# ICLDisco/parsec

Measured on NVIDIA H100. Metric: tasks/s, higher is better.
Workload: dtype i32

## Files before the change

include/pb2_engine.h:

```cpp
#ifndef PB2_ENGINE_H
#define PB2_ENGINE_H

#include <stddef.h>
#include <stdint.h>

#ifdef __cplusplus
extern "C" {
#endif

#define PB2_SUCCESS                   0
#define PB2_ERROR                    -1
#define PB2_ERR_OUT_OF_RESOURCE      -2
#define PB2_ERR_NOT_FOUND            -3
#define PB2_ERR_BAD_PARAM            -4
#define PB2_ERR_EXISTS               -5
#define PB2_ERR_NOT_IMPLEMENTED      -6
#define PB2_ERR_NOT_SUPPORTED        -7
#define PB2_ERR_VALUE_OUT_OF_BOUNDS  -8
#define PB2_ERR_TRUNCATE             -9
#define PB2_ERR_DEVICE              -10

#define PB2_FLOW_ACCESS_NONE   0x00
#define PB2_FLOW_ACCESS_READ   0x04
#define PB2_FLOW_ACCESS_WRITE  0x08
// ... 56 lines not shown
} pb2_tile_t;

#define PB2_SRC_HOST 0
#define PB2_SRC_PEER 1
#define PB2_SRC_PUSH 2

#define PB2_TILE_INVALID   0
#define PB2_TILE_STAGING   1
#define PB2_TILE_VALID     2

typedef struct pb2_engine_params_s {
    int32_t  workers_per_sm;
    int32_t  threads;
    int32_t  max_workers;
    int32_t  stage_mode;
    int32_t  queue_policy;
    int32_t  timeout_ms;
    int32_t  gemm_mode;
    int32_t  part_bytes;
    int32_t  read_groups;
    int32_t  fuse_readers;
} pb2_engine_params_t;

typedef struct pb2_engine_info_s {
    int32_t  cuda_device;
    int32_t  sm_count;
    int32_t  cc_major, cc_minor;
    int32_t  nworkers;
    int32_t  nworkers_gemm;
    int32_t  can_map_host;
    int32_t  reserved;
    uint64_t total_mem;
    uint64_t free_mem;
} pb2_engine_info_t;

typedef struct pb2_window_stats_s {
    uint64_t tasks_retired;
    uint64_t bytes_h2d;
    uint64_t bytes_d2d;
    uint64_t bytes_d2h;
    uint64_t stage_ins;
    uint64_t body_errors;
    float    kernel_ms;
    float    reset_ms;
} pb2_window_stats_t;

typedef struct pb2_engine_s pb2_engine_t;
typedef struct pb2_window_s pb2_window_t;

int  pb2_engine_create(pb2_engine_t** engine, int cuda_device, const pb2_engine_params_t* params);
int  pb2_engine_destroy(pb2_engine_t* engine);
int  pb2_engine_info(pb2_engine_t* engine, pb2_engine_info_t* info);
const char* pb2_engine_last_error(pb2_engine_t* engine);

int  pb2_engine_malloc(pb2_engine_t* engine, size_t bytes, void** dev_ptr);
int  pb2_engine_free(pb2_engine_t* engine, void* dev_ptr);
int  pb2_engine_host_register(pb2_engine_t* engine, void* host_ptr, size_t bytes, void** dev_alias);
int  pb2_engine_host_unregister(pb2_engine_t* engine, void* host_ptr);
int  pb2_engine_memcpy_h2d(pb2_engine_t* engine, void* dev, const void* host, size_t bytes);
int  pb2_engine_prefetch_h2d(pb2_engine_t* engine, void* dev, size_t dev_pitch, const void* host, size_t host_pitch,
                             size_t width_bytes, size_t rows);
int  pb2_engine_memcpy_d2h(pb2_engine_t* engine, void* host, const void* dev, size_t bytes);
int  pb2_engine_synchronize(pb2_engine_t* engine);
int  pb2_engine_set_stream(pb2_engine_t* engine, void* cuda_stream);
void* pb2_engine_get_stream(pb2_engine_t* engine);

int  pb2_engine_copy_batch(pb2_engine_t* engine, void* const* dst, const void* const* src, const uint64_t* bytes, int32_t n);

int  pb2_engine_ipc_export(pb2_engine_t* engine, void* dev_ptr, unsigned char handle[64]);
int  pb2_engine_ipc_open(pb2_engine_t* engine, const unsigned char handle[64], void** dev_ptr);
int  pb2_engine_ipc_close(pb2_engine_t* engine, void* dev_ptr);
int  pb2_engine_enable_peer(pb2_engine_t* engine, int peer_cuda_device);
int  pb2_body_launch(void* cuda_stream, int body, int nb_args, void* const* ptrs, const uint64_t* bytes,
                     const int32_t* iparam3, float fparam);
int  pb2_body_launch_errors(uint64_t* errors, int reset);
int  pb2_engine_set_shared_windows(pb2_engine_t* engine, int on, const int32_t* next_rs_begin);
int  pb2_engine_set_part_bytes(pb2_engine_t* engine, int32_t part_bytes);
int  pb2_engine_set_window_trace(pb2_engine_t* engine, int on);
int  pb2_engine_set_stage_slice_bytes(pb2_engine_t* engine, int32_t bytes);

#define PB2_IMAGE_PTX   1
#define PB2_IMAGE_CUBIN 2
int  pb2_engine_link_bodies(pb2_engine_t* engine, const void* image, size_t bytes, int format, uint32_t sliceable);
int  pb2_engine_link_bodies_checked(pb2_engine_t* engine, const void* image, size_t bytes, int format, uint32_t sliceable,
                                    uint32_t checked);
#define PB2_LINK_GEMM_WINDOWS 0x1u
#define PB2_LINK_READERS(mask) ((uint32_t)(mask) << 8)
#define PB2_LINK_READER_GROUPS(mask) ((uint32_t)(mask) << 16)
// ... 89 lines not shown
```

parsec_b200/_lib.py:

```python
import ctypes as C
import os

import numpy as np

_HERE = os.path.dirname(os.path.abspath(__file__))
LIB_PATH = os.environ.get("PB2_LIB_PATH") or os.path.join(_HERE, "libparsec_b200.so")

PB2_SUCCESS = 0
PB2_ERROR = -1
PB2_ERR_OUT_OF_RESOURCE = -2
PB2_ERR_NOT_FOUND = -3
PB2_ERR_BAD_PARAM = -4
PB2_ERR_EXISTS = -5
PB2_ERR_NOT_IMPLEMENTED = -6
PB2_ERR_NOT_SUPPORTED = -7
PB2_ERR_VALUE_OUT_OF_BOUNDS = -8
PB2_ERR_TRUNCATE = -9
PB2_ERR_DEVICE = -10

ERR_NAMES = {
    0: "PB2_SUCCESS", -1: "PB2_ERROR", -2: "PB2_ERR_OUT_OF_RESOURCE", -3: "PB2_ERR_NOT_FOUND",
    -4: "PB2_ERR_BAD_PARAM", -5: "PB2_ERR_EXISTS", -6: "PB2_ERR_NOT_IMPLEMENTED",
    -7: "PB2_ERR_NOT_SUPPORTED", -8: "PB2_ERR_VALUE_OUT_OF_BOUNDS", -9: "PB2_ERR_TRUNCATE",
    -10: "PB2_ERR_DEVICE",
}

ACCESS_NONE, ACCESS_READ, ACCESS_WRITE, ACCESS_RW, FLOW_PUSHOUT = 0x00, 0x04, 0x08, 0x0C, 0x40

BODY_NOP, BODY_FILL_I32, BODY_CHECK_I32, BODY_INCR_I32, BODY_ADD_IOTA_I32 = 0, 1, 2, 3, 4
BODY_SCALE_I32, BODY_IOTA_I32, BODY_COPY, BODY_FILL_F32, BODY_CHECK_F32 = 5, 6, 7, 8, 9
BODY_INCR_F32, BODY_AXPY_F32, BODY_MEMSET_U8, BODY_ADD_AT_I32, BODY_GEMM_BF16 = 10, 11, 12, 13, 16
BODY_LINKED_0, BODY_LINKED_7 = 20, 27
IMAGE_PTX, IMAGE_CUBIN = 1, 2
LINK_GEMM_WINDOWS = 0x1


def LINK_READERS(mask):
    return mask << 8


def LINK_READER_GROUPS(mask):
    return mask << 16


def LINK_GEMM_BODIES(mask):
    return mask << 24

TASK_DEPS_MASK = 0x01
TILE_INVALID, TILE_STAGING, TILE_VALID = 0, 1, 2
SRC_HOST, SRC_PEER = 0, 1
MAX_FLOWS = 4

TASK_DTYPE = np.dtype([
    ("dep_goal", "<i4"), ("succ_begin", "<i4"), ("succ_count", "<i4"), ("priority", "<i4"),
    ("body", "u1"), ("nb_flows", "u1"), ("flags", "u1"), ("class_id", "u1"),
    ("tile", "<i4", (4,)), ("access", "u1", (4,)),
    ("iparam", "<i4", (3,)), ("fparam", "<f4"), ("locals", "<i4", (2,)),
], align=False)
assert TASK_DTYPE.itemsize == 64

TILE_DTYPE = np.dtype([
    ("dev_ptr", "<u8"), ("src_ptr", "<u8"), ("bytes", "<u4"), ("state", "<i4"),
    ("version", "<u4"), ("src_kind", "<i4"),
], align=False)
assert TILE_DTYPE.itemsize == 32

PART_WAITED_INPUT, PART_RETIRED = 1, 2
PART_TRACE_DTYPE = np.dtype([
    ("t_pop_ns", "<u8"), ("t_in_ns", "<u8"), ("t_exec_ns", "<u8"), ("t_out_ns", "<u8"),
    ("in_bytes", "<u8"), ("out_bytes", "<u8"), ("task", "<i4"), ("part", "<u2"), ("nparts", "<u2"),
    ("smid", "<u4"), ("flags", "<u4"),
], align=False)
assert PART_TRACE_DTYPE.itemsize == 64

BODY_ARGS_DTYPE = np.dtype([
    ("flow", "<u8", (4,)), ("bytes", "<u4", (4,)), ("elem0", "<u4"), ("part", "<u4"),
    ("iparam", "<i4", (3,)), ("fparam", "<f4"),
], align=True)
assert BODY_ARGS_DTYPE.itemsize == 72


def succ_make(task, flow=0):
    return (np.uint32(flow) << np.uint32(27)) | np.uint32(task)


class EngineParams(C.Structure):
    _fields_ = [("workers_per_sm", C.c_int32), ("threads", C.c_int32), ("max_workers", C.c_int32),
                ("stage_mode", C.c_int32), ("queue_policy", C.c_int32), ("timeout_ms", C.c_int32),
                ("gemm_mode", C.c_int32), ("part_bytes", C.c_int32), ("read_groups", C.c_int32),
                ("fuse_readers", C.c_int32)]


class EngineInfo(C.Structure):
    _fields_ = [("cuda_device", C.c_int32), ("sm_count", C.c_int32), ("cc_major", C.c_int32),
                ("cc_minor", C.c_int32), ("nworkers", C.c_int32), ("nworkers_gemm", C.c_int32),
                ("can_map_host", C.c_int32), ("reserved", C.c_int32),
                ("total_mem", C.c_uint64), ("free_mem", C.c_uint64)]


class WindowStats(C.Structure):
    _fields_ = [("tasks_retired", C.c_uint64), ("bytes_h2d", C.c_uint64), ("bytes_d2d", C.c_uint64),
                ("bytes_d2h", C.c_uint64), ("stage_ins", C.c_uint64), ("body_errors", C.c_uint64),
                ("kernel_ms", C.c_float), ("reset_ms", C.c_float)]


class WindowHandle(C.Structure):
    _fields_ = [("dep", C.c_ubyte * 64), ("ring", C.c_ubyte * 64), ("ctl", C.c_ubyte * 64), ("tiles", C.c_ubyte * 64),
                ("cap_mask", C.c_uint32), ("ntasks", C.c_int32), ("entry_kind", C.c_int32), ("ntiles", C.c_int32)]


PUSH_DTYPE = np.dtype([("dst", np.uint64), ("bytes", np.uint32), ("src_tile", np.int32), ("rank", np.int32), ("desc", np.int32),
                       ("pad", np.int32, (2,))])
assert PUSH_DTYPE.itemsize == 32


class PartitionSizes(C.Structure):
    _fields_ = [("ntasks", C.c_int32), ("nsucc", C.c_int32), ("ntiles", C.c_int32), ("nready", C.c_int32),
                ("nremote", C.c_int32), ("nslots", C.c_int32), ("slab_bytes", C.c_uint64)]


class Pb2Error(RuntimeError):
    def __init__(self, rc, what, detail=""):
        self.rc = rc
        super().__init__(f"{what}: {ERR_NAMES.get(rc, rc)} {detail}".strip())


_lib = None

ENGINE_SYMBOLS = [
    "pb2_engine_create", "pb2_engine_destroy", "pb2_engine_info", "pb2_engine_last_error",
    "pb2_engine_malloc", "pb2_engine_free", "pb2_engine_host_register", "pb2_engine_host_unregister",
    "pb2_engine_memcpy_h2d", "pb2_engine_prefetch_h2d", "pb2_engine_memcpy_d2h", "pb2_engine_synchronize", "pb2_engine_set_stream", "pb2_engine_get_stream", "pb2_engine_copy_batch", "pb2_engine_ipc_export", "pb2_engine_ipc_open",
    "pb2_engine_ipc_close", "pb2_engine_enable_peer", "pb2_body_launch", "pb2_body_launch_errors", "pb2_engine_set_shared_windows", "pb2_engine_set_part_bytes", "pb2_engine_set_window_trace", "pb2_engine_set_stage_slice_bytes", "pb2_window_export", "pb2_window_set_remote", "pb2_window_task_entries",
    "pb2_window_arm", "pb2_window_start",
    "pb2_window_create", "pb2_window_destroy", "pb2_window_launch", "pb2_window_wait",
    "pb2_window_results", "pb2_window_trace", "pb2_window_part_trace",
    "pb2_partition_create", "pb2_partition_sizes", "pb2_partition_get", "pb2_partition_destroy", "pb2_partition_error",
    "pb2_partition_set_push", "pb2_partition_push_count", "pb2_partition_get_push", "pb2_window_set_push",
    "pb2_engine_link_bodies", "pb2_engine_link_bodies_checked", "pb2_engine_linked_info",
    "pb2_engine_link_bodies_ex", "pb2_engine_linked_gemm_info",
]


def load():
    global _lib
    if _lib is not None:
        return _lib
    if not os.path.exists(LIB_PATH):
        raise ImportError(
            f"{LIB_PATH} is missing: run `make` (or __graft_entry__.build()) first. "
            "parsec_b200 has no CPU fallback.")
    lib = C.CDLL(LIB_PATH)
    vp, i32, u64 = C.c_void_p, C.c_int32, C.c_uint64
    P = C.POINTER
    lib.pb2_engine_create.argtypes = [P(vp), C.c_int, P(EngineParams)]
    lib.pb2_engine_destroy.argtypes = [vp]
    lib.pb2_engine_info.argtypes = [vp, P(EngineInfo)]
    lib.pb2_engine_last_error.argtypes = [vp]
    lib.pb2_engine_last_error.restype = C.c_char_p
    lib.pb2_engine_malloc.argtypes = [vp, C.c_size_t, P(vp)]
    lib.pb2_engine_free.argtypes = [vp, vp]
    lib.pb2_engine_host_register.argtypes = [vp, vp, C.c_size_t, P(vp)]
    lib.pb2_engine_host_unregister.argtypes = [vp, vp]
    lib.pb2_engine_memcpy_h2d.argtypes = [vp, vp, vp, C.c_size_t]
    lib.pb2_engine_memcpy_d2h.argtypes = [vp, vp, vp, C.c_size_t]
    lib.pb2_engine_synchronize.argtypes = [vp]
    lib.pb2_engine_set_stream.argtypes = [vp, vp]
    lib.pb2_engine_copy_batch.argtypes = [vp, vp, vp, vp, i32]
    lib.pb2_engine_ipc_export.argtypes = [vp, vp, vp]
    lib.pb2_engine_ipc_open.argtypes = [vp, vp, P(vp)]
    lib.pb2_engine_ipc_close.argtypes = [vp, vp]
    lib.pb2_engine_enable_peer.argtypes = [vp, C.c_int]
    lib.pb2_body_launch.argtypes = [vp, C.c_int, C.c_int, vp, vp, vp, C.c_float]
    lib.pb2_body_launch_errors.argtypes = [vp, C.c_int]
    lib.pb2_engine_set_shared_windows.argtypes = [vp, C.c_int, vp]
    lib.pb2_window_task_entries.argtypes = [vp, vp]
    lib.pb2_engine_set_part_bytes.argtypes = [vp, i32]
    lib.pb2_engine_set_window_trace.argtypes = [vp, C.c_int]
    lib.pb2_window_trace.argtypes = [vp, vp, vp, vp, vp]
    lib.pb2_window_part_trace.argtypes = [vp, vp, i32, P(i32)]
    lib.pb2_engine_set_stage_slice_bytes.argtypes = [vp, i32]
    lib.pb2_engine_link_bodies.argtypes = [vp, C.c_char_p, C.c_size_t, C.c_int, C.c_uint32]
    lib.pb2_engine_link_bodies_checked.argtypes = [vp, C.c_char_p, C.c_size_t, C.c_int, C.c_uint32, C.c_uint32]
    lib.pb2_engine_linked_info.argtypes = [vp, P(i32), P(i32), P(i32), P(i32)]
    lib.pb2_engine_link_bodies_ex.argtypes = [vp, C.c_char_p, C.c_size_t, C.c_int, C.c_uint32, C.c_uint32, C.c_uint32]
    lib.pb2_engine_linked_gemm_info.argtypes = [vp, P(i32), P(i32), P(i32), P(i32)]
    lib.pb2_window_export.argtypes = [vp, vp]
    lib.pb2_window_set_remote.argtypes = [vp, i32, i32, vp, vp, vp, vp, i32]
    lib.pb2_partition_set_push.argtypes = [vp, C.c_int]
    lib.pb2_partition_push_count.argtypes = [vp, i32, vp]
    lib.pb2_partition_get_push.argtypes = [vp, i32, vp, vp, vp]
    lib.pb2_window_set_push.argtypes = [vp, vp, vp, i32]
    lib.pb2_window_arm.argtypes = [vp]
# ... 20 lines not shown
```

parsec_b200/csrc/pb2_engine.cu:

```cuda
#include <cuda_runtime.h>
#include <cuda.h>
#include <stdio.h>
#include <stdlib.h>
#include <string.h>
#include <string>
#include <vector>
#include <mutex>
#include <map>
#include <algorithm>
#include <type_traits>

#include "../../include/pb2_engine.h"
#include "pb2_sched.cuh"
#include "pb2_hbm.cuh"
#include "pb2_gemm.cuh"

namespace pb2 {

__global__ void pb2_window_reset_kernel(Win2Dev g, const pb2_tile_t* tiles_init,
                                        const int32_t* ready, int32_t nready) {
    const size_t gid = (size_t)blockIdx.x * blockDim.x + threadIdx.x;
    const size_t gsz = (size_t)gridDim.x * blockDim.x;
    for (size_t i = gid; i < (size_t)g.nunits; i += gsz) { g.udep[i] = g.units[i].dep_goal; g.parts_left[i] = g.units[i].nparts; }
    if (g.trace.parts)
// ... 206 lines not shown
static int read_part_records(pb2_window_t* w, std::vector<pb2_part_trace_t>& out) {
    pb2_engine_t* e = w->e;
    std::vector<pb2_part_trace_t> rec((size_t)w->shape.part_records);
    out.clear();
    if (rec.empty()) return PB2_SUCCESS;
    PB2_CUDA(e, cudaSetDevice(e->cuda_device));
    PB2_CUDA(e, cudaMemcpy(rec.data(), run_desc(w, w->cur).trace.parts, rec.size() * sizeof(pb2_part_trace_t), cudaMemcpyDeviceToHost));
    out.reserve(rec.size());
    for (const PartEntity& pe : w->part_entities)
        for (int32_t p = 0; p < pe.nparts; ++p) {
            out.push_back(rec[(size_t)(pe.base + p)]);
            out.back().task = pe.lead; out.back().part = (uint16_t)p; out.back().nparts = (uint16_t)pe.nparts;
        }
    return PB2_SUCCESS;
}

extern "C" const unsigned char pb2_linked_engine_image[], pb2_linked_engine_image_end[];
extern "C" const unsigned char pb2_linked_gemm_image[], pb2_linked_gemm_image_end[];
extern "C" const unsigned char pb2_linked_engine_groups_image[], pb2_linked_engine_groups_image_end[];
extern "C" const unsigned char pb2_linked_gemm_groups_image[], pb2_linked_gemm_groups_image_end[];

static const char* const kLinkedKernels[2][4] = {
    {"_ZN3pb221pb2_engine_hbm_kernelILb0ELb0ELb1EEEvNS_6WinDevENS_8TraceDevE",
     "_ZN3pb221pb2_engine_hbm_kernelILb1ELb0ELb1EEEvNS_6WinDevENS_8TraceDevE",
     "_ZN3pb221pb2_engine_hbm_kernelILb0ELb1ELb1EEEvNS_6WinDevENS_8TraceDevE",
     "_ZN3pb221pb2_engine_hbm_kernelILb1ELb1ELb1EEEvNS_6WinDevENS_8TraceDevE"},
    {"_ZN3pb223pb2_engine_gemm2_kernelILb0ELb0ELb1EEEvNS_7Win2DevE",
     "_ZN3pb223pb2_engine_gemm2_kernelILb1ELb0ELb1EEEvNS_7Win2DevE",
     "_ZN3pb223pb2_engine_gemm2_kernelILb0ELb1ELb1EEEvNS_7Win2DevE",
     "_ZN3pb223pb2_engine_gemm2_kernelILb1ELb1ELb1EEEvNS_7Win2DevE"},
};

struct DriverCalls {
    decltype(&cuLinkCreate) link_create = nullptr;
    decltype(&cuLinkAddData) link_add = nullptr;
    decltype(&cuLinkComplete) link_complete = nullptr;
    decltype(&cuLinkDestroy) link_destroy = nullptr;
    decltype(&cuModuleLoadData) module_load = nullptr;
    decltype(&cuModuleUnload) module_unload = nullptr;
    decltype(&cuModuleGetFunction) get_function = nullptr;
    decltype(&cuFuncGetAttribute) func_attr = nullptr;
    decltype(&cuFuncSetAttribute) func_set_attr = nullptr;
    decltype(&cuOccupancyMaxActiveBlocksPerMultiprocessor) occupancy = nullptr;
    decltype(&cuLaunchKernel) launch = nullptr;
    bool complete() const {
        return link_create && link_add && link_complete && link_destroy && module_load && module_unload && get_function &&
               func_attr && func_set_attr && occupancy && launch;
    }
};

static const DriverCalls& driver() {
    static const DriverCalls d = [] {
        DriverCalls r;
        auto get = [](const char* name, auto& fn) {
            void* p = nullptr;
            cudaDriverEntryPointQueryResult q;
            if (cudaGetDriverEntryPoint(name, &p, cudaEnableDefault, &q) == cudaSuccess && q == cudaDriverEntryPointSuccess)
                fn = reinterpret_cast<std::remove_reference_t<decltype(fn)>>(p);
        };
        get("cuLinkCreate", r.link_create); get("cuLinkAddData", r.link_add); get("cuLinkComplete", r.link_complete);
        get("cuLinkDestroy", r.link_destroy); get("cuModuleLoadData", r.module_load); get("cuModuleUnload", r.module_unload);
        get("cuModuleGetFunction", r.get_function); get("cuFuncGetAttribute", r.func_attr);
        get("cuFuncSetAttribute", r.func_set_attr);
        get("cuOccupancyMaxActiveBlocksPerMultiprocessor", r.occupancy); get("cuLaunchKernel", r.launch);
        return r;
    }();
    return d;
}

static CUresult resolve_kernel(const pb2_engine_t* e, CUfunction fn, int kind, bool linked, WindowKernel& k, bool& fits) {
    const DriverCalls& d = driver();
    const bool gemm = kind == 1;
    const int workers = gemm ? e->nworkers_gemm : e->nworkers;
    k = WindowKernel{};
    k.fn = fn;
    k.block = gemm ? gemm::kThreads : (unsigned)e->params.threads;
    k.dyn_smem = gemm ? gemm::kSmemBytes : 0;
    fits = true;
    CUresult r = d.func_attr(&k.regs, CU_FUNC_ATTRIBUTE_NUM_REGS, fn);
    if (r == CUDA_SUCCESS) r = d.func_attr(&k.local, CU_FUNC_ATTRIBUTE_LOCAL_SIZE_BYTES, fn);
    if (r == CUDA_SUCCESS) r = d.func_attr(&k.static_smem, CU_FUNC_ATTRIBUTE_SHARED_SIZE_BYTES, fn);
    if (r != CUDA_SUCCESS) return r;
    if (gemm && d.func_set_attr(fn, CU_FUNC_ATTRIBUTE_MAX_DYNAMIC_SHARED_SIZE_BYTES, gemm::kSmemBytes) != CUDA_SUCCESS) {
        fits = false;
        return CUDA_SUCCESS;
    }
    int occ = 0;
    r = d.occupancy(&occ, fn, (int)k.block, k.dyn_smem);
    if (r == CUDA_SUCCESS && gemm && occ == 0) fits = false;
    k.grid = (unsigned)(linked ? std::max(1, std::min(workers, e->prop.multiProcessorCount * occ)) : workers);
    return r;
}

static int window_kernel(pb2_engine_t* e, bool linked, int kind, int v, WindowKernel& out) {
    static WindowKernelSymbols (*const symbols[4])() = {window_kernels_0, window_kernels_1, window_kernels_2, window_kernels_3};
    std::lock_guard<std::mutex> lk(e->mu);
    WindowKernel& k = e->kernels[linked ? 1 : 0][kind][v];
    if (!k.fn && !linked) {
        if (!driver().complete()) { e->last_error = "the driver's kernel entry points are not available"; return PB2_ERR_NOT_SUPPORTED; }
        const WindowKernelSymbols s = symbols[v]();
// ... 124 lines not shown
    int ndev = 0;
    cudaError_t err = cudaGetDeviceCount(&ndev);
    if (err != cudaSuccess || ndev == 0) {
        fprintf(stderr, "pb2_engine_create: no CUDA device (%s)\n", cudaGetErrorString(err));
        return PB2_ERR_DEVICE;
    }
    if (cuda_device < 0 || cuda_device >= ndev) return PB2_ERR_BAD_PARAM;
    pb2_engine_t* e = new pb2_engine_s();
    e->cuda_device = cuda_device;
    PB2_CUDA(e, cudaSetDevice(cuda_device));
    PB2_CUDA(e, cudaGetDeviceProperties(&e->prop, cuda_device));
    if (e->prop.major != 9 || e->prop.minor != 0) {
        fprintf(stderr, "pb2_engine_create: device %d is sm_%d%d; this library only carries sm_90a code\n",
                cuda_device, e->prop.major, e->prop.minor);
        delete e;
        return PB2_ERR_NOT_SUPPORTED;
    }
    pb2_engine_params_t p{};
    if (params) p = *params;
    if (p.workers_per_sm <= 0) p.workers_per_sm = kHbmWorkersPerSm;
    if (p.threads <= 0 || p.threads > PB2_HBM_THREADS) p.threads = PB2_HBM_THREADS;
    p.threads = (p.threads + 31) & ~31;
    if (p.timeout_ms <= 0) p.timeout_ms = 20000;
    if (p.part_bytes == 0) p.part_bytes = kDefaultPartBytes;
    e->params = p;
    if (const char* sl = getenv("PB2_STAGE_SLICE_BYTES")) e->stage_slice_bytes = atoi(sl);
    if (const char* sm = getenv("PB2_STAGE_MODE")) e->params.stage_mode = atoi(sm);
    PB2_CUDA(e, cudaStreamCreateWithFlags(&e->own_stream, cudaStreamNonBlocking));
    PB2_CUDA(e, cudaStreamCreateWithFlags(&e->up_stream, cudaStreamNonBlocking));
    PB2_CUDA(e, cudaStreamCreateWithFlags(&e->dma_stream, cudaStreamNonBlocking));
    PB2_CUDA(e, cudaStreamCreateWithFlags(&e->arm_stream, cudaStreamNonBlocking));
    PB2_CUDA(e, cudaEventCreateWithFlags(&e->dma_ev, cudaEventDisableTiming));
    e->stream = e->own_stream;
    {
        cudaMemPool_t pool;
        if (cudaDeviceGetDefaultMemPool(&pool, cuda_device) == cudaSuccess) {
            unsigned long long thr = ~0ull;
            cudaMemPoolSetAttribute(pool, cudaMemPoolAttrReleaseThreshold, &thr);
        }
    }
    int occ = 0;
    PB2_CUDA(e, cudaOccupancyMaxActiveBlocksPerMultiprocessor(&occ, window_kernels_0().hbm, p.threads, 0));
    int per_sm = occ < p.workers_per_sm ? occ : p.workers_per_sm;
    if (per_sm < 1) per_sm = 1;
    e->nworkers = e->prop.multiProcessorCount * per_sm;
    if (p.max_workers > 0 && p.max_workers < e->nworkers) e->nworkers = p.max_workers;
    e->nworkers_gemm = e->prop.multiProcessorCount;
    if (p.max_workers > 0 && p.max_workers < e->nworkers_gemm) e->nworkers_gemm = p.max_workers;
    *engine = e;
    return PB2_SUCCESS;
}

int pb2_engine_destroy(pb2_engine_t* e) {
    if (!e) return PB2_ERR_BAD_PARAM;
    cudaSetDevice(e->cuda_device);
    for (auto& kv : e->registered) cudaHostUnregister(kv.first);
    if (e->own_stream) cudaStreamDestroy(e->own_stream);
    if (e->up_stream) cudaStreamDestroy(e->up_stream);
    if (e->dma_stream) cudaStreamDestroy(e->dma_stream);
    if (e->arm_stream) cudaStreamDestroy(e->arm_stream);
    if (e->dma_ev) cudaEventDestroy(e->dma_ev);
    if (e->linked_module) driver().module_unload(e->linked_module);
    delete e;
    return PB2_SUCCESS;
}

int pb2_engine_info(pb2_engine_t* e, pb2_engine_info_t* info) {
    if (!e || !info) return PB2_ERR_BAD_PARAM;
    memset(info, 0, sizeof *info);
    info->cuda_device = e->cuda_device;
    info->sm_count = e->prop.multiProcessorCount;
    info->cc_major = e->prop.major; info->cc_minor = e->prop.minor;
    info->nworkers = e->nworkers; info->nworkers_gemm = e->nworkers_gemm;
    info->can_map_host = e->prop.canMapHostMemory;
    size_t f = 0, t = 0;
    PB2_CUDA(e, cudaSetDevice(e->cuda_device));
    PB2_CUDA(e, cudaMemGetInfo(&f, &t));
    info->total_mem = t; info->free_mem = f;
    return PB2_SUCCESS;
}

const char* pb2_engine_last_error(pb2_engine_t* e) { return e ? e->last_error.c_str() : "null engine"; }

int pb2_engine_malloc(pb2_engine_t* e, size_t bytes, void** dev_ptr) {
    if (!e || !dev_ptr) return PB2_ERR_BAD_PARAM;
    PB2_CUDA(e, cudaSetDevice(e->cuda_device));
    cudaError_t err = cudaMalloc(dev_ptr, bytes ? bytes : 16);
    if (err == cudaErrorMemoryAllocation) { cudaGetLastError(); *dev_ptr = nullptr; return PB2_ERR_OUT_OF_RESOURCE; }
    PB2_CUDA(e, err);
    return PB2_SUCCESS;
}

int pb2_engine_free(pb2_engine_t* e, void* dev_ptr) {
    if (!e) return PB2_ERR_BAD_PARAM;
    PB2_CUDA(e, cudaSetDevice(e->cuda_device));
    PB2_CUDA(e, cudaFree(dev_ptr));
    return PB2_SUCCESS;
}

int pb2_engine_host_register(pb2_engine_t* e, void* host_ptr, size_t bytes, void** dev_alias) {
    if (!e || !host_ptr || !bytes) return PB2_ERR_BAD_PARAM;
    std::lock_guard<std::mutex> lk(e->mu);
    auto it = e->registered.find(host_ptr);
    if (it != e->registered.end()) {
        if (dev_alias) *dev_alias = it->second.second;
        return PB2_SUCCESS;
    }
    PB2_CUDA(e, cudaSetDevice(e->cuda_device));
    cudaError_t err = cudaHostRegister(host_ptr, bytes, cudaHostRegisterPortable | cudaHostRegisterMapped);
    if (err == cudaErrorHostMemoryAlreadyRegistered) { cudaGetLastError(); }
    else PB2_CUDA(e, err);
    void* alias = nullptr;
    PB2_CUDA(e, cudaHostGetDevicePointer(&alias, host_ptr, 0));
    if (err != cudaErrorHostMemoryAlreadyRegistered) e->registered[host_ptr] = {bytes, alias};
    if (dev_alias) *dev_alias = alias;
    return PB2_SUCCESS;
}

int pb2_engine_host_unregister(pb2_engine_t* e, void* host_ptr) {
    if (!e) return PB2_ERR_BAD_PARAM;
    std::lock_guard<std::mutex> lk(e->mu);
    auto it = e->registered.find(host_ptr);
    if (it == e->registered.end()) return PB2_ERR_NOT_FOUND;
    PB2_CUDA(e, cudaSetDevice(e->cuda_device));
    PB2_CUDA(e, cudaHostUnregister(host_ptr));
    e->registered.erase(it);
    return PB2_SUCCESS;
}

// ... 15 lines not shown
    e->dma_pending = true;
    return PB2_SUCCESS;
}

int pb2_engine_memcpy_d2h(pb2_engine_t* e, void* host, const void* dev, size_t bytes) {
    if (!e) return PB2_ERR_BAD_PARAM;
    PB2_CUDA(e, cudaSetDevice(e->cuda_device));
    PB2_CUDA(e, cudaMemcpyAsync(host, dev, bytes, cudaMemcpyDeviceToHost, e->stream));
    PB2_CUDA(e, cudaStreamSynchronize(e->stream));
    return PB2_SUCCESS;
}

int pb2_engine_copy_batch(pb2_engine_t* e, void* const* dst, const void* const* src, const uint64_t* bytes, int32_t n) {
    if (!e || n < 0 || (n && (!dst || !src || !bytes))) return PB2_ERR_BAD_PARAM;
    if (n == 0) return PB2_SUCCESS;
    for (int32_t i = 0; i < n; ++i)
        if (bytes[i] >= (1ull << 32)) { e->last_error = "copy of 4 GiB or more"; return PB2_ERR_VALUE_OUT_OF_BOUNDS; }
    PB2_CUDA(e, cudaSetDevice(e->cuda_device));
    std::vector<CopyDesc> h((size_t)n);
    for (int32_t i = 0; i < n; ++i) h[i] = CopyDesc{dst[i], src[i], bytes[i]};
    CopyDesc* d = nullptr;
    PB2_CUDA(e, cudaMallocAsync(reinterpret_cast<void**>(&d), sizeof(CopyDesc) * (size_t)n, e->stream));
    PB2_CUDA(e, cudaMemcpyAsync(d, h.data(), sizeof(CopyDesc) * (size_t)n, cudaMemcpyHostToDevice, e->stream));
    PB2_CUDA(e, cudaStreamSynchronize(e->stream));
    const int grid = n < e->nworkers ? n : e->nworkers;
    pb2_copy_batch_kernel<<<grid, 256, 0, e->stream>>>(d, n);
    PB2_CUDA(e, cudaGetLastError());
    PB2_CUDA(e, cudaFreeAsync(d, e->stream));
    return PB2_SUCCESS;
}

int pb2_engine_ipc_export(pb2_engine_t* e, void* dev_ptr, unsigned char handle[64]) {
    if (!e || !dev_ptr || !handle) return PB2_ERR_BAD_PARAM;
    PB2_CUDA(e, cudaSetDevice(e->cuda_device));
    cudaIpcMemHandle_t ih;
    PB2_CUDA(e, cudaIpcGetMemHandle(&ih, dev_ptr));
    memcpy(handle, &ih, 64);
    return PB2_SUCCESS;
}
int pb2_engine_ipc_open(pb2_engine_t* e, const unsigned char handle[64], void** dev_ptr) {
    if (!e || !dev_ptr || !handle) return PB2_ERR_BAD_PARAM;
    PB2_CUDA(e, cudaSetDevice(e->cuda_device));
    cudaIpcMemHandle_t ih;
    memcpy(&ih, handle, 64);
    PB2_CUDA(e, cudaIpcOpenMemHandle(dev_ptr, ih, cudaIpcMemLazyEnablePeerAccess));
    return PB2_SUCCESS;
}
int pb2_engine_ipc_close(pb2_engine_t* e, void* dev_ptr) {
    if (!e || !dev_ptr) return PB2_ERR_BAD_PARAM;
    PB2_CUDA(e, cudaSetDevice(e->cuda_device));
    PB2_CUDA(e, cudaIpcCloseMemHandle(dev_ptr));
    return PB2_SUCCESS;
}
int pb2_engine_enable_peer(pb2_engine_t* e, int peer_cuda_device) {
    if (!e) return PB2_ERR_BAD_PARAM;
    if (peer_cuda_device == e->cuda_device) return PB2_SUCCESS;
    PB2_CUDA(e, cudaSetDevice(e->cuda_device));
    int can = 0;
    PB2_CUDA(e, cudaDeviceCanAccessPeer(&can, e->cuda_device, peer_cuda_device));
    if (!can) return PB2_ERR_NOT_SUPPORTED;
    cudaError_t err = cudaDeviceEnablePeerAccess(peer_cuda_device, 0);
    if (err == cudaErrorPeerAccessAlreadyEnabled) { cudaGetLastError(); return PB2_SUCCESS; }
    PB2_CUDA(e, err);
    return PB2_SUCCESS;
}

// ... 380 lines not shown
```

parsec_b200/csrc/pb2_engine_priv.hpp:

```cpp
#pragma once
#include <cuda.h>
#include <cuda_runtime.h>
#include <stdio.h>
#include <map>
#include <mutex>
#include <string>
#include <utility>
#include "../../include/pb2_engine.h"
#include "pb2_window_layout.h"

struct WindowKernel {
    CUfunction fn = nullptr;
    unsigned grid = 0, block = 0, dyn_smem = 0;
    int32_t regs = 0, local = 0, static_smem = 0;
};

struct WindowKernelSymbols { const void* hbm; const void* gemm; };
WindowKernelSymbols window_kernels_0();
WindowKernelSymbols window_kernels_1();
WindowKernelSymbols window_kernels_2();
WindowKernelSymbols window_kernels_3();

struct pb2_engine_s {
    int cuda_device = 0;
    cudaDeviceProp prop{};
    pb2_engine_params_t params{};
    cudaStream_t stream = nullptr;
    cudaStream_t own_stream = nullptr;
    cudaStream_t up_stream = nullptr;
    cudaStream_t dma_stream = nullptr;
    cudaStream_t arm_stream = nullptr;
    cudaEvent_t dma_ev = nullptr;
    bool dma_pending = false;
    int nworkers = 0;
    int32_t stage_slice_bytes = 64 * 1024;
    int nworkers_gemm = 0;
    std::string last_error;
    std::mutex mu;
    bool shared_windows = false;
    bool window_trace = false;
    const int32_t* next_rs_begin = nullptr;
    std::map<void*, std::pair<size_t, void*>> registered;
    WindowKernel kernels[2][2][4];
    CUmodule linked_module = nullptr;
    uint32_t linked_sliceable = 0, linked_checked = 0, linked_readers = 0, linked_reader_groups = 0, linked_gemm_bodies = 0;
};

static inline uint32_t link_readers(uint32_t flags) { return (flags >> 8) & 0xFFu; }
static inline uint32_t link_reader_groups(uint32_t flags) { return (flags >> 16) & 0xFFu; }

static inline uint32_t link_gemm_bodies(uint32_t flags) { return (flags >> 24) & 0xFFu; }

static inline const char* link_args_error(const void* image, size_t bytes, int format, uint32_t sliceable, uint32_t checked,
                                          uint32_t flags = 0) {
    if (flags & ~(uint32_t)(PB2_LINK_GEMM_WINDOWS | PB2_LINK_READERS(0xFFu) | PB2_LINK_READER_GROUPS(0xFFu) |
                            PB2_LINK_GEMM_BODIES(0xFFu)))
        return "link flags have an unknown bit (PB2_LINK_GEMM_WINDOWS, PB2_LINK_READERS(mask), bits 8..15, "
               "PB2_LINK_READER_GROUPS(mask), bits 16..23, and PB2_LINK_GEMM_BODIES(mask), bits 24..31, are the only flags)";
    if (!image || !bytes) return "linked body image is NULL or empty";
    if (format != PB2_IMAGE_PTX && format != PB2_IMAGE_CUBIN) return "linked body image format must be PB2_IMAGE_PTX or PB2_IMAGE_CUBIN";
    if (sliceable >> 8) return "sliceable mask has bits above bit 7 (there are 8 linked body ids)";
    if (checked >> 8) return "checked mask has bits above bit 7 (there are 8 linked body ids)";
    if (checked & ~sliceable) return "checked mask has a bit that is clear in the sliceable mask (a checked body must be sliceable)";
    if (link_readers(flags) & ~sliceable) return "readers mask has a bit that is clear in the sliceable mask (a reader must be sliceable)";
    if (link_reader_groups(flags) & ~link_readers(flags))
        return "link flags have an unknown bit: the reader groups mask has a bit that is clear in the readers mask (only a "
               "reader has the group form)";
    if (link_gemm_bodies(flags) && !(flags & PB2_LINK_GEMM_WINDOWS))
        return "GEMM-worker bodies mask without PB2_LINK_GEMM_WINDOWS (a GEMM-worker body runs in GEMM windows only)";
    if (link_gemm_bodies(flags) & sliceable)
        return "GEMM-worker bodies mask has a bit that is set in the sliceable mask (a GEMM-worker body runs as one part; "
               "it can be neither checked nor a reader)";
    return nullptr;
}

// ... 14 lines not shown
```

parsec_b200/engine.py:

```python
import ctypes as C

import numpy as np

from . import _lib as L


def _check(rc, what, engine=None):
    if rc != L.PB2_SUCCESS:
        detail = ""
        if engine is not None and engine._h:
            detail = (L.load().pb2_engine_last_error(engine._h) or b"").decode()
        raise L.Pb2Error(rc, what, detail)


def _ptr(a):
    return None if a is None else a.ctypes.data_as(C.c_void_p)


def chrome_trace(t_start_ns, t_end_ns, smid, class_id=None, locals=None, class_names=None, unit=None, pid=0,
                 process_name=None):
    t0 = np.asarray(t_start_ns, np.uint64)
    t1 = np.asarray(t_end_ns, np.uint64)
    sm = np.asarray(smid, np.uint32)
    rec = np.nonzero(t1 != 0)[0]
# ... 42 lines not shown
        t = [int(r["t_pop_ns"]), int(r["t_in_ns"]), int(r["t_exec_ns"]), int(r["t_out_ns"])]
        for (name, t0, t1, nbytes) in (("movein", t[0], t[1], int(r["in_bytes"])), (body, t[1], t[2], None),
                                       ("moveout", t[2], t[3], int(r["out_bytes"]))):
            if t1 <= t0:
                continue
            a = dict(args) if nbytes is None else dict(args, bytes=nbytes)
            events.append({"ph": "X", "name": name, "pid": pid, "tid": int(r["smid"]),
                           "ts": (t0 - base) / 1000.0, "dur": (t1 - t0) / 1000.0, "args": a})
    return {"traceEvents": events, "displayTimeUnit": "ns"}


class Engine:

    def __init__(self, cuda_device=0, workers_per_sm=0, threads=0, max_workers=0, stage_mode=0,
                 queue_policy=0, timeout_ms=0, gemm_mode=0, part_bytes=0, read_groups=0,
                 fuse_readers=0, window_trace=False):
        self._lib = L.load()
        self._h = C.c_void_p()
        p = L.EngineParams(workers_per_sm, threads, max_workers, stage_mode, queue_policy, timeout_ms, gemm_mode, part_bytes,
                           read_groups, fuse_readers)
        rc = self._lib.pb2_engine_create(C.byref(self._h), cuda_device, C.byref(p))
        if rc != L.PB2_SUCCESS:
            self._h = C.c_void_p()
            raise L.Pb2Error(rc, "pb2_engine_create")
        self._allocs = []
        if window_trace:
            self.set_window_trace(True)

    def info(self):
        i = L.EngineInfo()
        _check(self._lib.pb2_engine_info(self._h, C.byref(i)), "pb2_engine_info", self)
        return {f[0]: getattr(i, f[0]) for f in L.EngineInfo._fields_ if f[0] != "reserved"}

    def malloc(self, nbytes):
        p = C.c_void_p()
        _check(self._lib.pb2_engine_malloc(self._h, nbytes, C.byref(p)), "pb2_engine_malloc", self)
        self._allocs.append(p.value)
        return p.value

    def free(self, ptr):
        _check(self._lib.pb2_engine_free(self._h, C.c_void_p(ptr)), "pb2_engine_free", self)
        if ptr in self._allocs:
            self._allocs.remove(ptr)

    def host_register(self, arr):
        alias = C.c_void_p()
        _check(self._lib.pb2_engine_host_register(self._h, _ptr(arr), arr.nbytes, C.byref(alias)),
               "pb2_engine_host_register", self)
        return alias.value

    def host_unregister(self, arr):
        _check(self._lib.pb2_engine_host_unregister(self._h, _ptr(arr)), "pb2_engine_host_unregister", self)

    def h2d(self, dev_ptr, arr):
        arr = np.ascontiguousarray(arr)
        _check(self._lib.pb2_engine_memcpy_h2d(self._h, C.c_void_p(dev_ptr), _ptr(arr), arr.nbytes), "h2d", self)
        self.synchronize()

    def d2h(self, arr, dev_ptr):
        assert arr.flags["C_CONTIGUOUS"]
        _check(self._lib.pb2_engine_memcpy_d2h(self._h, _ptr(arr), C.c_void_p(dev_ptr), arr.nbytes), "d2h", self)
        return arr

    def use_stream(self, cuda_stream):
        if not cuda_stream:
            raise ValueError("use_stream needs a real stream handle (the legacy default stream is 0: create a torch.cuda.Stream)")
        _check(self._lib.pb2_engine_set_stream(self._h, C.c_void_p(cuda_stream)), "pb2_engine_set_stream", self)

    def set_shared_windows(self, on=True, next_rs_begin=None):
# ... 167 lines not shown
```

parsec_b200/multigpu.py:

```python
import ctypes as C
import os

import numpy as np

from . import _lib as L


class Partition:

    def __init__(self, tasks, succ, tiles, ready, task_rank, tile_rank, nranks, part_bytes=0):
        self._lib = L.load()
        self._h = C.c_void_p()
        tasks = np.ascontiguousarray(tasks, L.TASK_DTYPE)
        succ = np.ascontiguousarray(succ, np.uint32)
        tiles = np.ascontiguousarray(tiles, L.TILE_DTYPE)
        ready = np.ascontiguousarray(ready, np.int32)
        task_rank = np.ascontiguousarray(task_rank, np.int32)
        tile_rank = np.ascontiguousarray(tile_rank, np.int32)
        assert len(task_rank) == len(tasks) and len(tile_rank) == len(tiles)
        vp = lambda a: a.ctypes.data_as(C.c_void_p)
        rc = self._lib.pb2_partition_create(C.byref(self._h), vp(tasks), len(tasks), vp(succ), len(succ), vp(tiles), len(tiles),
                                            vp(ready), len(ready), vp(task_rank), vp(tile_rank), nranks, part_bytes)
        if rc != L.PB2_SUCCESS:
            raise L.Pb2Error(rc, "pb2_partition_create", (self._lib.pb2_partition_error() or b"").decode())
# ... 168 lines not shown
        begin[i] = len(succ)
        for d, f in es:
            succ.append((f << 27) | d)
            goal[d] |= 1 << f
    t["succ_begin"], t["succ_count"], t["dep_goal"] = begin, [len(e) for e in edges], goal
    tiles = np.zeros(ntiles, L.TILE_DTYPE)
    tiles["bytes"], tiles["state"] = nb * nb * elem_bytes, L.TILE_VALID
    mm = np.array([m for m in range(NT) for n in range(m + 1)])
    nn = np.array([n for m in range(NT) for n in range(m + 1)])
    tile_rank = ((mm % P) * Q + (nn % Q)).astype(np.int32)
    rw_tile = np.array([r[5][-1][0] for r in rows])
    ready = np.nonzero(goal == 0)[0].astype(np.int32)
    return t, np.array(succ, np.uint32), tiles, ready, tile_rank[rw_tile].astype(np.int32), tile_rank


def translate_remote_targets(part, entries_by_rank):
    tgt = part["rs_target"].copy()
    for r, table in enumerate(entries_by_rank):
        m = part["rs_rank"] == r
        if m.any():
            tgt[m] = np.asarray(table)[part["rs_target"][m].astype(np.int64)].astype(np.uint32)
    return tgt


class SharedRun:

    def __init__(self, eng, part, rank, world, dist, torch, kind=0, push=None):
        self.eng, self.rank, self.world, self.dist, self.torch = eng, rank, world, dist, torch
        if push is None:
            push = (kind == 0) and os.environ.get("PB2_MGPU_PUSH", "0") == "1"
        part.set_push(push)
        z = part.sizes(rank)
        self.slab_bytes = max(int(z["slab_bytes"]), 256)
        self.slab = eng.malloc(self.slab_bytes)
        eng.h2d(self.slab, np.zeros(self.slab_bytes, np.uint8))
        eng.synchronize()
        handles = [None] * world
        dist.all_gather_object(handles, eng.ipc_export(self.slab))
        self.base = [self.slab if r == rank else eng.ipc_open(handles[r]) for r in range(world)]
        self.p = part.get(rank, self.base)
        eng.set_shared_windows(True, self.p["rs_begin"])
        self.w = eng.window(kind, self.p["tasks"], self.p["succ"], self.p["tiles"], self.p["ready"])
        eng.set_shared_windows(False)
        wh = [None] * world
        dist.all_gather_object(wh, (self.w.export(), self.w.task_entries()))
        tgt = translate_remote_targets(self.p, [h[1] for h in wh])
        self.w.set_remote(rank, [h[0] for h in wh], self.p["rs_begin"], self.p["rs_rank"], tgt)
        self.npush = 0
        if push:
            ps_begin, pushes = part.get_push(rank, self.base)
            self.npush = len(pushes)
            self.w.set_push(ps_begin, pushes)
        self._flag = torch.zeros(1, dtype=torch.int32, device="cuda")
        dist.barrier()

    def slot_of(self, tile):
        hit = np.nonzero(self.p["slot_tile"] == tile)[0]
        if not len(hit):
            return None
        return self.slab + int(self.p["slot_offset"][int(hit[0])])

    def load_home_tiles(self, tile_rank, data):
        for tile in np.nonzero(np.asarray(tile_rank) == self.rank)[0]:
            addr = self.slot_of(int(tile))
            if addr is not None:
                self.eng.h2d(addr, np.ascontiguousarray(data[int(tile)]))
        self.eng.synchronize()
# ... 150 lines not shown
```

Measured before the change: 99.47 million.

## Allocate device buffers with generic compressible memory via VMM when supported

Adds a driver-API path that allocates device memory with CU_MEM_ALLOCATION_COMP_GENERIC through cuMemCreate/cuMemMap whenever the device reports compression support and the request is at least one granule. The aim is to cut DRAM bandwidth for compressible data such as zero-filled or uniform i32 tiles. IPC slabs opt out because CUDA IPC cannot export such memory. Freeing now forces a device synchronize, and allocation goes through a mutex. Devices without generic compression support (H100 may be one) fall back to cudaMalloc.

```diff
diff --git a/include/pb2_engine.h b/include/pb2_engine.h
--- a/include/pb2_engine.h
+++ b/include/pb2_engine.h
@@ -112,6 +112,8 @@
     int32_t  reserved;
     uint64_t total_mem;
     uint64_t free_mem;
+    int32_t  compression_supported;
+    int32_t  slab_compressible;
 } pb2_engine_info_t;
 
 typedef struct pb2_window_stats_s {
@@ -133,7 +135,9 @@
 int  pb2_engine_info(pb2_engine_t* engine, pb2_engine_info_t* info);
 const char* pb2_engine_last_error(pb2_engine_t* engine);
 
+#define PB2_MALLOC_IPC 0x1u
 int  pb2_engine_malloc(pb2_engine_t* engine, size_t bytes, void** dev_ptr);
+int  pb2_engine_malloc_ex(pb2_engine_t* engine, size_t bytes, uint32_t flags, void** dev_ptr);
 int  pb2_engine_free(pb2_engine_t* engine, void* dev_ptr);
 int  pb2_engine_host_register(pb2_engine_t* engine, void* host_ptr, size_t bytes, void** dev_alias);
 int  pb2_engine_host_unregister(pb2_engine_t* engine, void* host_ptr);
diff --git a/parsec_b200/_lib.py b/parsec_b200/_lib.py
--- a/parsec_b200/_lib.py
+++ b/parsec_b200/_lib.py
@@ -33,6 +33,7 @@
 BODY_LINKED_0, BODY_LINKED_7 = 20, 27
 IMAGE_PTX, IMAGE_CUBIN = 1, 2
 LINK_GEMM_WINDOWS = 0x1
+MALLOC_IPC = 0x1
 
 
 def LINK_READERS(mask):
@@ -95,7 +96,8 @@
     _fields_ = [("cuda_device", C.c_int32), ("sm_count", C.c_int32), ("cc_major", C.c_int32),
                 ("cc_minor", C.c_int32), ("nworkers", C.c_int32), ("nworkers_gemm", C.c_int32),
                 ("can_map_host", C.c_int32), ("reserved", C.c_int32),
-                ("total_mem", C.c_uint64), ("free_mem", C.c_uint64)]
+                ("total_mem", C.c_uint64), ("free_mem", C.c_uint64),
+                ("compression_supported", C.c_int32), ("slab_compressible", C.c_int32)]
 
 
 class WindowStats(C.Structure):
@@ -129,7 +131,7 @@
 
 ENGINE_SYMBOLS = [
     "pb2_engine_create", "pb2_engine_destroy", "pb2_engine_info", "pb2_engine_last_error",
-    "pb2_engine_malloc", "pb2_engine_free", "pb2_engine_host_register", "pb2_engine_host_unregister",
+    "pb2_engine_malloc", "pb2_engine_malloc_ex", "pb2_engine_free", "pb2_engine_host_register", "pb2_engine_host_unregister",
     "pb2_engine_memcpy_h2d", "pb2_engine_prefetch_h2d", "pb2_engine_memcpy_d2h", "pb2_engine_synchronize", "pb2_engine_set_stream", "pb2_engine_get_stream", "pb2_engine_copy_batch", "pb2_engine_ipc_export", "pb2_engine_ipc_open",
     "pb2_engine_ipc_close", "pb2_engine_enable_peer", "pb2_body_launch", "pb2_body_launch_errors", "pb2_engine_set_shared_windows", "pb2_engine_set_part_bytes", "pb2_engine_set_window_trace", "pb2_engine_set_stage_slice_bytes", "pb2_window_export", "pb2_window_set_remote", "pb2_window_task_entries",
     "pb2_window_arm", "pb2_window_start",
@@ -159,6 +161,7 @@
     lib.pb2_engine_last_error.argtypes = [vp]
     lib.pb2_engine_last_error.restype = C.c_char_p
     lib.pb2_engine_malloc.argtypes = [vp, C.c_size_t, P(vp)]
+    lib.pb2_engine_malloc_ex.argtypes = [vp, C.c_size_t, C.c_uint32, P(vp)]
     lib.pb2_engine_free.argtypes = [vp, vp]
     lib.pb2_engine_host_register.argtypes = [vp, vp, C.c_size_t, P(vp)]
     lib.pb2_engine_host_unregister.argtypes = [vp, vp]
diff --git a/parsec_b200/csrc/pb2_engine.cu b/parsec_b200/csrc/pb2_engine.cu
--- a/parsec_b200/csrc/pb2_engine.cu
+++ b/parsec_b200/csrc/pb2_engine.cu
@@ -262,6 +262,21 @@
 };
 
 struct DriverCalls {
+    decltype(&cuDeviceGet) device_get = nullptr;
+    decltype(&cuDeviceGetAttribute) device_attr = nullptr;
+    decltype(&cuMemCreate) mem_create = nullptr;
+    decltype(&cuMemGetAllocationGranularity) mem_granularity = nullptr;
+    decltype(&cuMemGetAllocationPropertiesFromHandle) mem_props = nullptr;
+    decltype(&cuMemAddressReserve) mem_reserve = nullptr;
+    decltype(&cuMemMap) mem_map = nullptr;
+    decltype(&cuMemSetAccess) mem_set_access = nullptr;
+    decltype(&cuMemUnmap) mem_unmap = nullptr;
+    decltype(&cuMemAddressFree) mem_address_free = nullptr;
+    decltype(&cuMemRelease) mem_release = nullptr;
+    bool vmm() const {
+        return device_get && device_attr && mem_create && mem_granularity && mem_props && mem_reserve && mem_map &&
+               mem_set_access && mem_unmap && mem_address_free && mem_release;
+    }
     decltype(&cuLinkCreate) link_create = nullptr;
     decltype(&cuLinkAddData) link_add = nullptr;
     decltype(&cuLinkComplete) link_complete = nullptr;
@@ -293,9 +308,74 @@
         get("cuModuleGetFunction", r.get_function); get("cuFuncGetAttribute", r.func_attr);
         get("cuFuncSetAttribute", r.func_set_attr);
         get("cuOccupancyMaxActiveBlocksPerMultiprocessor", r.occupancy); get("cuLaunchKernel", r.launch);
+        get("cuDeviceGet", r.device_get); get("cuDeviceGetAttribute", r.device_attr); get("cuMemCreate", r.mem_create);
+        get("cuMemGetAllocationGranularity", r.mem_granularity);
+        get("cuMemGetAllocationPropertiesFromHandle", r.mem_props); get("cuMemAddressReserve", r.mem_reserve);
+        get("cuMemMap", r.mem_map); get("cuMemSetAccess", r.mem_set_access); get("cuMemUnmap", r.mem_unmap);
+        get("cuMemAddressFree", r.mem_address_free); get("cuMemRelease", r.mem_release);
         return r;
     }();
     return d;
+}
+
+static CUmemAllocationProp compressible_prop(int dev) {
+    CUmemAllocationProp p{};
+    p.type = CU_MEM_ALLOCATION_TYPE_PINNED;
+    p.location.type = CU_MEM_LOCATION_TYPE_DEVICE;
+    p.location.id = dev;
+    p.allocFlags.compressionType = CU_MEM_ALLOCATION_COMP_GENERIC;
+    return p;
+}
+
+static size_t compressible_granule(int dev) {
+    const DriverCalls& d = driver();
+    CUdevice cd = 0;
+    int on = 0;
+    size_t g = 0;
+    if (!d.vmm() || d.device_get(&cd, dev) != CUDA_SUCCESS ||
+        d.device_attr(&on, CU_DEVICE_ATTRIBUTE_GENERIC_COMPRESSION_SUPPORTED, cd) != CUDA_SUCCESS || !on)
+        return 0;
+    const CUmemAllocationProp p = compressible_prop(dev);
+    return d.mem_granularity(&g, &p, CU_MEM_ALLOC_GRANULARITY_MINIMUM) == CUDA_SUCCESS ? g : 0;
+}
+
+static void release_compressible(void* p, CUmemGenericAllocationHandle h, size_t bytes, bool mapped = true) {
+    const DriverCalls& d = driver();
+    const CUdeviceptr ptr = reinterpret_cast<CUdeviceptr>(p);
+    if (mapped) d.mem_unmap(ptr, bytes);
+    if (ptr) d.mem_address_free(ptr, bytes);
+    d.mem_release(h);
+}
+
+static void* map_compressible(pb2_engine_t* e, size_t bytes, CUmemGenericAllocationHandle& h) {
+    const DriverCalls& d = driver();
+    const CUmemAllocationProp p = compressible_prop(e->cuda_device);
+    if (d.mem_create(&h, bytes, &p, 0) != CUDA_SUCCESS) return nullptr;
+    CUmemAllocationProp got{};
+    CUdeviceptr ptr = 0;
+    bool mapped = false;
+    bool ok = d.mem_props(&got, h) == CUDA_SUCCESS && got.allocFlags.compressionType == CU_MEM_ALLOCATION_COMP_GENERIC;
+    if (ok) ok = d.mem_reserve(&ptr, bytes, e->comp_granule, 0, 0) == CUDA_SUCCESS;
+    if (ok) ok = mapped = d.mem_map(ptr, bytes, 0, h, 0) == CUDA_SUCCESS;
+    if (ok) {
+        int ndev = 0;
+        if (cudaGetDeviceCount(&ndev) != cudaSuccess) { cudaGetLastError(); ndev = 0; }
+        std::vector<CUmemAccessDesc> access;
+        for (int dev = 0; dev < ndev; ++dev) {
+            int can = dev == e->cuda_device;
+            if (!can && cudaDeviceCanAccessPeer(&can, dev, e->cuda_device) != cudaSuccess) { cudaGetLastError(); can = 0; }
+            if (can != 1) continue;
+            CUmemAccessDesc a{};
+            a.location.type = CU_MEM_LOCATION_TYPE_DEVICE;
+            a.location.id = dev;
+            a.flags = CU_MEM_ACCESS_FLAGS_PROT_READWRITE;
+            access.push_back(a);
+        }
+        ok = !access.empty() && d.mem_set_access(ptr, bytes, access.data(), access.size()) == CUDA_SUCCESS;
+    }
+    if (ok) return reinterpret_cast<void*>(ptr);
+    release_compressible(reinterpret_cast<void*>(ptr), h, bytes, mapped);
+    return nullptr;
 }
 
 static CUresult resolve_kernel(const pb2_engine_t* e, CUfunction fn, int kind, bool linked, WindowKernel& k, bool& fits) {
@@ -486,6 +566,7 @@
     PB2_CUDA(e, cudaStreamCreateWithFlags(&e->arm_stream, cudaStreamNonBlocking));
     PB2_CUDA(e, cudaEventCreateWithFlags(&e->dma_ev, cudaEventDisableTiming));
     e->stream = e->own_stream;
+    e->comp_granule = compressible_granule(cuda_device);
     {
         cudaMemPool_t pool;
         if (cudaDeviceGetDefaultMemPool(&pool, cuda_device) == cudaSuccess) {
@@ -515,6 +596,8 @@
     if (e->arm_stream) cudaStreamDestroy(e->arm_stream);
     if (e->dma_ev) cudaEventDestroy(e->dma_ev);
     if (e->linked_module) driver().module_unload(e->linked_module);
+    if (!e->compressible.empty()) cudaDeviceSynchronize();
+    for (auto& kv : e->compressible) release_compressible(kv.first, kv.second.first, kv.second.second);
     delete e;
     return PB2_SUCCESS;
 }
@@ -531,14 +614,31 @@
     PB2_CUDA(e, cudaSetDevice(e->cuda_device));
     PB2_CUDA(e, cudaMemGetInfo(&f, &t));
     info->total_mem = t; info->free_mem = f;
+    info->compression_supported = e->comp_granule != 0;
+    info->slab_compressible = e->slab_compressible;
     return PB2_SUCCESS;
 }
 
 const char* pb2_engine_last_error(pb2_engine_t* e) { return e ? e->last_error.c_str() : "null engine"; }
 
-int pb2_engine_malloc(pb2_engine_t* e, size_t bytes, void** dev_ptr) {
-    if (!e || !dev_ptr) return PB2_ERR_BAD_PARAM;
-    PB2_CUDA(e, cudaSetDevice(e->cuda_device));
+int pb2_engine_malloc(pb2_engine_t* e, size_t bytes, void** dev_ptr) { return pb2_engine_malloc_ex(e, bytes, 0, dev_ptr); }
+
+int pb2_engine_malloc_ex(pb2_engine_t* e, size_t bytes, uint32_t flags, void** dev_ptr) {
+    if (!e || !dev_ptr || (flags & ~PB2_MALLOC_IPC)) return PB2_ERR_BAD_PARAM;
+    PB2_CUDA(e, cudaSetDevice(e->cuda_device));
+    const size_t g = e->comp_granule;
+    if (g && bytes >= g) {
+        std::lock_guard<std::mutex> lk(e->mu);
+        const size_t mapped = (bytes + g - 1) / g * g;
+        CUmemGenericAllocationHandle h{};
+        void* p = (flags & PB2_MALLOC_IPC) ? nullptr : map_compressible(e, mapped, h);
+        e->slab_compressible = p != nullptr;
+        if (p) {
+            e->compressible[p] = {h, mapped};
+            *dev_ptr = p;
+            return PB2_SUCCESS;
+        }
+    }
     cudaError_t err = cudaMalloc(dev_ptr, bytes ? bytes : 16);
     if (err == cudaErrorMemoryAllocation) { cudaGetLastError(); *dev_ptr = nullptr; return PB2_ERR_OUT_OF_RESOURCE; }
     PB2_CUDA(e, err);
@@ -548,7 +648,18 @@
 int pb2_engine_free(pb2_engine_t* e, void* dev_ptr) {
     if (!e) return PB2_ERR_BAD_PARAM;
     PB2_CUDA(e, cudaSetDevice(e->cuda_device));
-    PB2_CUDA(e, cudaFree(dev_ptr));
+    std::unique_lock<std::mutex> lk(e->mu);
+    auto it = e->compressible.find(dev_ptr);
+    if (it == e->compressible.end()) {
+        lk.unlock();
+        PB2_CUDA(e, cudaFree(dev_ptr));
+        return PB2_SUCCESS;
+    }
+    const auto [h, bytes] = it->second;
+    e->compressible.erase(it);
+    lk.unlock();
+    PB2_CUDA(e, cudaDeviceSynchronize());
+    release_compressible(dev_ptr, h, bytes);
     return PB2_SUCCESS;
 }
 
@@ -630,6 +741,16 @@
 
 int pb2_engine_ipc_export(pb2_engine_t* e, void* dev_ptr, unsigned char handle[64]) {
     if (!e || !dev_ptr || !handle) return PB2_ERR_BAD_PARAM;
+    {
+        std::lock_guard<std::mutex> lk(e->mu);
+        auto it = e->compressible.upper_bound(dev_ptr);
+        if (it != e->compressible.begin() &&
+            static_cast<char*>(dev_ptr) < static_cast<char*>(std::prev(it)->first) + std::prev(it)->second.second) {
+            e->last_error = "the memory is compressible, which CUDA IPC cannot export: allocate memory for other processes "
+                            "with pb2_engine_malloc_ex(..., PB2_MALLOC_IPC, ...)";
+            return PB2_ERR_NOT_SUPPORTED;
+        }
+    }
     PB2_CUDA(e, cudaSetDevice(e->cuda_device));
     cudaIpcMemHandle_t ih;
     PB2_CUDA(e, cudaIpcGetMemHandle(&ih, dev_ptr));
diff --git a/parsec_b200/csrc/pb2_engine_priv.hpp b/parsec_b200/csrc/pb2_engine_priv.hpp
--- a/parsec_b200/csrc/pb2_engine_priv.hpp
+++ b/parsec_b200/csrc/pb2_engine_priv.hpp
@@ -41,6 +41,9 @@
     bool window_trace = false;
     const int32_t* next_rs_begin = nullptr;
     std::map<void*, std::pair<size_t, void*>> registered;
+    size_t comp_granule = 0;
+    std::map<void*, std::pair<CUmemGenericAllocationHandle, size_t>> compressible;
+    bool slab_compressible = false;
     WindowKernel kernels[2][2][4];
     CUmodule linked_module = nullptr;
     uint32_t linked_sliceable = 0, linked_checked = 0, linked_readers = 0, linked_reader_groups = 0, linked_gemm_bodies = 0;
diff --git a/parsec_b200/engine.py b/parsec_b200/engine.py
--- a/parsec_b200/engine.py
+++ b/parsec_b200/engine.py
@@ -98,9 +98,9 @@
         _check(self._lib.pb2_engine_info(self._h, C.byref(i)), "pb2_engine_info", self)
         return {f[0]: getattr(i, f[0]) for f in L.EngineInfo._fields_ if f[0] != "reserved"}
 
-    def malloc(self, nbytes):
+    def malloc(self, nbytes, ipc=False):
         p = C.c_void_p()
-        _check(self._lib.pb2_engine_malloc(self._h, nbytes, C.byref(p)), "pb2_engine_malloc", self)
+        _check(self._lib.pb2_engine_malloc_ex(self._h, nbytes, L.MALLOC_IPC if ipc else 0, C.byref(p)), "pb2_engine_malloc_ex", self)
         self._allocs.append(p.value)
         return p.value
 
diff --git a/parsec_b200/multigpu.py b/parsec_b200/multigpu.py
--- a/parsec_b200/multigpu.py
+++ b/parsec_b200/multigpu.py
@@ -224,7 +224,7 @@
         part.set_push(push)
         z = part.sizes(rank)
         self.slab_bytes = max(int(z["slab_bytes"]), 256)
-        self.slab = eng.malloc(self.slab_bytes)
+        self.slab = eng.malloc(self.slab_bytes, ipc=True)
         eng.h2d(self.slab, np.zeros(self.slab_bytes, np.uint8))
         eng.synchronize()
         handles = [None] * world
```

New measurement: 121.7 million (median of 6 runs). 1.22x the previous value.
